# YuyangSunshine/ABR_IOD

Hardware: AMD Instinct MI355X
Metric: training images/sec (R50-C4 Faster R-CNN + ARD) (higher is better)
Workload: dtype f32 (tensors, accumulation and error bound; contractions via a 2-term fp16 split of both operands scaled by their amax, 3 cross products on the fp16 matrix cores: f16x3)

## Files before the change

abr_iod_amd/_lib.py:

```python
import ctypes as C
import os

import torch

_HERE = os.path.dirname(os.path.abspath(__file__))
LIB_PATH = os.environ.get("ABR_IOD_HIP_LIB") or os.path.join(_HERE, "libabr_iod_hip.so")

NCHW, NHWC = 0, 1

_vp, _i, _f, _i64 = C.c_void_p, C.c_int, C.c_float, C.c_int64


class ConvDesc(C.Structure):

    _fields_ = [
        ("B", _i), ("H", _i), ("W", _i), ("Cin", _i),
        ("Cout", _i), ("R", _i), ("S", _i),
        ("stride", _i), ("pad", _i),
        ("Ho", _i), ("Wo", _i),
        ("scale", _vp), ("bias", _vp), ("residual", _vp), ("mask", _vp),
        ("relu", _i),
        ("out_H", _i), ("out_W", _i), ("out_sh", _i), ("out_sw", _i),
        ("math", _i),
        ("wino_v", _vp),
# ... 81 lines not shown
    "abr_deform_psroi_backward": (_i, [_vp, _vp, _vp, _vp, _vp, _vp, _i, _i, _i, _i, _i, _f, _i, _i, _i, _i, _i, _f, _i, _i, _vp, _vp, _vp, _vp]),
    "abr_nms_workspace_bytes": (_i64, [_i, _i]),
    "abr_nms_unsorted_workspace_bytes": (_i64, [_i]),
    "abr_nms": (_i, [_vp, _vp, _i, _f, _i, _vp, _vp, _vp, _i64, _vp]),
    "abr_sort_scores_max_n": (_i64, []),
    "abr_sort_scores_desc": (_i, [_vp, _i, _vp, _vp]),
    "abr_nms_sorted_batched": (_i, [_vp, _vp, _i, _i, _f, _i, _i, _vp, _vp, _vp, _i64, _vp]),
    "abr_roi_align_forward_f64": (_i, [_vp, _vp, _i, _i, _i, _i, _i, C.c_double, _i, _i, _i, _vp, _vp]),
    "abr_roi_align_backward_f64": (_i, [_vp, _vp, _i, _i, _i, _i, _i, C.c_double, _i, _i, _i, _vp, _vp]),
    "abr_sigmoid_focal_forward_f64": (_i, [_vp, _vp, _i, _i, _f, _f, _vp, _vp]),
    "abr_sigmoid_focal_backward_f64": (_i, [_vp, _vp, _vp, _i, _i, _f, _f, _vp, _vp]),
    "abr_sigmoid_focal_forward": (_i, [_vp, _vp, _i, _i, _f, _f, _vp, _vp]),
    "abr_sigmoid_focal_backward": (_i, [_vp, _vp, _vp, _i, _i, _f, _f, _vp, _vp]),
    "abr_ard_forward": (_i, [_vp, _vp, _i, _i, _i, _f, _i, _vp, _vp, _vp]),
    "abr_ard_backward": (_i, [_vp, _vp, _vp, _i, _i, _i, _f, _i, _f, _vp, _vp, _vp]),
    "abr_smooth_l1": (_i, [_vp, _vp, _i64, _f, _f, _vp, _f, _vp, _vp]),
    "abr_smooth_l1_rows": (_i, [_vp, _i, _vp, _vp, _vp, _vp, _i, _f, _f, _vp, _vp, _f, _vp, _vp]),
    "abr_softmax_ce": (_i, [_vp, _i, _vp, _i, _i, _i, _i, _vp, _f, _vp, _i, _vp]),
    "abr_feat_distill": (_i, [_vp, _vp, _i64, _vp, _vp, _f, _vp, _vp]),
    "abr_rpn_distill": (_i, [_vp, _vp, _i, _i, _vp, _vp, _i, _i, _i64, _i, _f, _i, _vp, _f, _vp, _vp, _i, _i, _vp]),
    "abr_roi_distill": (_i, [_vp, _vp, _vp, _vp, _i, _i, _i, _vp, _i, _vp, _f, _vp, _vp, _vp]),
    "abr_bce_logits_gather": (_i, [_vp, _vp, _vp, _vp, _i, _vp, _vp, _f, _vp, _vp]),
    "abr_img_resample_u8": (_i, [_vp, _i, _i, _vp, _i, _i, _vp, _vp, _i, _vp, _vp, _i, _vp, _vp]),
    "abr_img_blend_paste_u8": (_i, [_vp, _i, _i, _vp, _i, _i, _i, _i, _i, _i, _i, _i, C.c_double, _vp]),
    "abr_img_copy_rect_u8": (_i, [_vp, _i, _i, _vp, _i, _i, _i, _i, _i, _i, _i, _i, _vp]),
    "abr_img_fill_u8": (_i, [_vp, _i64, _i, _vp]),
    "abr_img_color_jitter_u8": (_i, [_vp, _i, _i, _i, C.c_double, _vp, _vp]),
    "abr_img_normalize_to_batch": (_i, [_vp, _i, _i, _i, _i, C.POINTER(C.c_float), C.POINTER(C.c_float), _vp, _i, _i, _vp]),
    "abr_conv_forward": (_i, [C.POINTER(ConvDesc), _vp, _vp, _vp, _vp]),
    "abr_conv_tail64_forward": (_i, [C.POINTER(ConvDesc), C.POINTER(ConvDesc), _vp, _vp, _vp, _vp, _vp]),
    "abr_conv_wgrad": (_i, [C.POINTER(ConvDesc), _vp, _vp, _vp, _vp]),
    "abr_conv_wino_v_floats": (_i64, [C.POINTER(ConvDesc)]),
    "abr_conv_route_info": (_i, [C.POINTER(ConvDesc), C.POINTER(C.c_int32)]),
    "abr_conv_packed_bytes": (_i64, [_i64, _i64]),
    "abr_conv_pack_weights": (_i, [_vp, _i64, _i, _vp, _vp]),
    "abr_conv_dgrad_weights": (_i, [_vp, _vp, _i, _i, _i, _i, _vp, _vp]),
    "abr_bias_grad": (_i, [_vp, _i64, _i, _vp, _vp]),
    "abr_nchw_to_nhwc_pad": (_i, [_vp, _i, _i, _i, _i, _i, _vp, _vp]),
    "abr_nchw_to_nhwc": (_i, [_vp, _i, _i, _i, _i, _vp, _vp]),
    "abr_nhwc_to_nchw": (_i, [_vp, _i, _i, _i, _i, _vp, _vp]),
    "abr_maxpool3x3s2": (_i, [_vp, _i, _i, _i, _i, _vp, _vp]),
    "abr_maxpool3x3s2_backward": (_i, [_vp, _vp, _i, _i, _i, _i, _vp, _vp]),
    "abr_deform_im2col": (_i, [_vp, _vp, _i, _i, _i, _i, _i, _i, _i, _vp, _vp]),
    "abr_deform_col2im_coord": (_i, [_vp, _vp, _vp, _i, _i, _i, _i, _i, _i, _i, _vp, _vp, _vp, C.c_uint32, _vp]),
    "abr_deform_im2col_general": (_i, [_vp, _vp, _vp] + [_i] * 16 + [_vp, _vp]),
    "abr_deform_col2im_coord_general": (_i, [_vp, _vp, _vp, _vp] + [_i] * 16 + [_vp, _vp, _vp, _vp]),
    "abr_avgpool_forward": (_i, [_vp, _i, _i, _i, _vp, _vp]),
    "abr_avgpool_backward": (_i, [_vp, _i, _i, _i, _vp, _vp]),
    "abr_avgpool_relu_backward": (_i, [_vp, _vp, _i, _i, _i, _vp, _vp]),
    "abr_avgpool_relu_backward_amax": (_i, [_vp, _vp, _i, _i, _i, _vp, _vp, C.c_uint32, _vp]),
    "abr_channel_mean": (_i, [_vp, _i64, _i, _vp, _vp]),
    "abr_relu_backward": (_i, [_vp, _vp, _i64, _vp, _vp]),
    "abr_add_inplace": (_i, [_vp, _vp, _i64, _vp]),
    "abr_scale_inplace": (_i, [_vp, _i64, _f, _vp, _vp]),
    "abr_grid_anchors": (_i, [_vp, _i, _i, _i, _i, _i, _i, _i, _vp, _vp, _vp]),
    "abr_topk_sigmoid": (_i, [_vp, _i64, _i, _i, _i, _i, _i, _vp, _vp, _vp]),
    "abr_det_softmax_decode": (_i, [_vp, _i, _vp, _i, _i, _i, _vp, _i, _i, _vp, _f, _f, _f, _f, _vp, _vp, _vp]),
    "abr_det_select_workspace_bytes": (_i64, [_i, _i, _i]),
    "abr_det_select": (_i, [_vp, _vp, _vp, _i, _i, _i, _f, _f, _i, _i, _vp, _vp, _vp, _vp, _vp, _vp, _vp, _vp, _i64, _vp]),
    "abr_rpn_decode_clip": (_i, [_vp, _i, _i, _i, _vp, _vp, _i, _i, _i, _vp, _f, _f, _f, _f, _vp, _vp]),
    "abr_rpn_pyramid_max_k": (_i, []),
    "abr_rpn_pyramid_topk": (_i, [_vp, _vp, _vp, _vp, _i, _i, _i, _i, _vp, _vp, _vp]),
    "abr_rpn_pyramid_decode": (_i, [_vp, _vp, _vp, _vp, _vp, _i, _i, _i, _i, _vp, _vp, _vp, _f, _f, _f, _f, _f, _vp, _vp, _vp, _vp]),
    "abr_rpn_pyramid_select": (_i, [_vp, _vp, _vp, _vp, _i, _i, _i, _i, _i, _i, _vp, _vp, _vp, _vp, _vp]),
    "abr_retina_max_candidates": (_i, []),
    "abr_retina_detect": (_i, [_vp, _vp, _vp, _vp, _vp, _vp, _i, _i, _i, _i, _vp, _f, _i, _f, _i, _f, _f, _f, _f, _f, _i, _vp, _vp, _vp, _vp, _vp]),
# ... 114 lines not shown
```

abr_iod_amd/csrc/conv_winograd.hip:

```cpp
#include <map>

#include <algorithm>
#include <map>
#include <functional>
#include <mutex>
#include <utility>
#include <type_traits>
#include <vector>

#include "common.h"

namespace {

template <int V>
struct vf {
    float v[V];
};
template <int V>
__device__ __forceinline__ vf<V> operator+(vf<V> a, vf<V> b) {
    vf<V> r;
#pragma unroll
    for (int i = 0; i < V; i++) r.v[i] = a.v[i] + b.v[i];
    return r;
}
template <int V>
__device__ __forceinline__ vf<V> operator-(vf<V> a, vf<V> b) {
    vf<V> r;
#pragma unroll
    for (int i = 0; i < V; i++) r.v[i] = a.v[i] - b.v[i];
    return r;
}
template <int V>
__device__ __forceinline__ vf<V> operator-(vf<V> a) {
    vf<V> r;
#pragma unroll
// ... 7 lines not shown
    for (int i = 0; i < V; i++) r.v[i] = s * a.v[i];
    return r;
}
template <int V>
__device__ __forceinline__ vf<V> vzero() {
    vf<V> r;
#pragma unroll
    for (int i = 0; i < V; i++) r.v[i] = 0.f;
    return r;
}
template <int V>
__device__ __forceinline__ vf<V> vld(const float* p);
template <>
__device__ __forceinline__ vf<2> vld<2>(const float* p) { const float2 t = *reinterpret_cast<const float2*>(p); return {{t.x, t.y}}; }
template <>
__device__ __forceinline__ vf<4> vld<4>(const float* p) { const float4 t = *reinterpret_cast<const float4*>(p); return {{t.x, t.y, t.z, t.w}}; }
template <int V>
__device__ __forceinline__ vf<V> vld_buf(__amdgpu_buffer_rsrc_t r, unsigned byte_off);
template <>
__device__ __forceinline__ vf<2> vld_buf<2>(__amdgpu_buffer_rsrc_t r, unsigned byte_off) {
    typedef unsigned u32x2 __attribute__((ext_vector_type(2)));
    const u32x2 t = __builtin_amdgcn_raw_buffer_load_b64(r, (int)byte_off, 0, 0);
    return {{__uint_as_float(t.x), __uint_as_float(t.y)}};
}
template <>
__device__ __forceinline__ vf<4> vld_buf<4>(__amdgpu_buffer_rsrc_t r, unsigned byte_off) {
    typedef unsigned u32x4 __attribute__((ext_vector_type(4)));
    const u32x4 t = __builtin_amdgcn_raw_buffer_load_b128(r, (int)byte_off, 0, 0);
    return {{__uint_as_float(t.x), __uint_as_float(t.y), __uint_as_float(t.z), __uint_as_float(t.w)}};
}
__device__ __forceinline__ void vst(float* p, vf<2> a) { *reinterpret_cast<float2*>(p) = make_float2(a.v[0], a.v[1]); }
__device__ __forceinline__ void vst(float* p, vf<4> a) { *reinterpret_cast<float4*>(p) = make_float4(a.v[0], a.v[1], a.v[2], a.v[3]); }

template <typename T>
__device__ __forceinline__ void bt6(const T d0, const T d1, const T d2, const T d3, const T d4, const T d5, T& o0, T& o1, T& o2, T& o3, T& o4,
                                    T& o5) {
    o0 = 4.f * d0 - 5.f * d2 + d4;
    o1 = d3 + d4 - 4.f * (d1 + d2);
    o2 = 4.f * d1 - 4.f * d2 - d3 + d4;
    o3 = 2.f * (d3 - d1) - d2 + d4;
    o4 = 2.f * d1 - d2 - 2.f * d3 + d4;
    o5 = 4.f * d1 - 5.f * d3 + d5;
}

template <int V>
__device__ __forceinline__ unsigned vabs_max(unsigned m, vf<V> a) {
#pragma unroll
    for (int i = 0; i < V; i++) m = max(m, __float_as_uint(a.v[i]) & 0x7FFFFFFFu);
    return m;
}

template <int V>
__global__ __launch_bounds__(256) void wino_input_kernel(const float* __restrict__ x, int B, int H, int W, int C, int th_n, int tw_n,
                                                         float* __restrict__ Vo, unsigned long long* amax, unsigned epoch) {
    unsigned am = 0;
    typedef vf<V> f2;
    const int64_t T = (int64_t)B * th_n * tw_n;
    const int C2 = C / V;
    const int64_t total = T * C2;
    const int64_t ps = T * C;
    const __amdgpu_buffer_rsrc_t rx = __builtin_amdgcn_make_buffer_rsrc(const_cast<float*>(x), 0, (unsigned)((int64_t)B * H * W * C * 4), 0x00020000);
    for (int64_t idx = (int64_t)blockIdx.x * blockDim.x + threadIdx.x; idx < total; idx += (int64_t)gridDim.x * blockDim.x) {
        const int c = V * (int)(idx % C2);
        const int64_t t = idx / C2;
        const int tw = (int)(t % tw_n), th = (int)((t / tw_n) % th_n), b = (int)(t / ((int64_t)tw_n * th_n));
        const int y0 = 4 * th - 1, x0 = 4 * tw - 1;
        f2 tcol[6][6];
        const int base = (b * H * W) * C + c;
#pragma unroll
        for (int j = 0; j < 6; j++) {
            const int xx = x0 + j;
            const bool xin = (unsigned)xx < (unsigned)W;
            f2 d[6];
#pragma unroll
            for (int i = 0; i < 6; i++) {
// ... 161 lines not shown
            const float4 a = *reinterpret_cast<const float4*>(src + (r * 3 + q) * 64), b = *reinterpret_cast<const float4*>(src + (r * 3 + q) * 64 + 4);
            gA[r][q] = {{a.x, a.y, a.z, a.w}};
            gB[r][q] = {{b.x, b.y, b.z, b.w}};
        }
    uint4* planes = reinterpret_cast<uint4*>(jb.dst);
    const float* scales = reinterpret_cast<const float*>(reinterpret_cast<const char*>(jb.dst) + abr::h3_planes_bytes_dev(36 * N, C));
    const int ks = kc * 4 + wave, KS = C / 16;
    auto emit = [&](int xi, const fv& uA, const fv& uB, float sc) {
        const float inv = 1.f / sc;
        unsigned h0[4], h1[4];
        abr::h3_split2(uA.v[0], uA.v[1], inv, h0[0], h1[0]);
        abr::h3_split2(uA.v[2], uA.v[3], inv, h0[1], h1[1]);
        abr::h3_split2(uB.v[0], uB.v[1], inv, h0[2], h1[2]);
        abr::h3_split2(uB.v[2], uB.v[3], inv, h0[3], h1[3]);
        const size_t nb = ((size_t)xi * N + n0) / 32;
        const size_t ch = (nb * KS + ks) * 2;
        planes[ch * 64 + lane] = make_uint4(h0[0], h0[1], h0[2], h0[3]);
        planes[(ch + 1) * 64 + lane] = make_uint4(h1[0], h1[1], h1[2], h1[3]);
    };
    auto row_i = [&](auto I) {
        constexpr int i = decltype(I)::value;
        float sc[6];
#pragma unroll
        for (int jj = 0; jj < 6; jj++) sc[jj] = scales[(size_t)(6 * i + jj) * N + n0 + row];
        fv uA[6], uB[6];
        wino_u_row<i>(gA, uA);
        wino_u_row<i>(gB, uB);
#pragma unroll
        for (int jj = 0; jj < 6; jj++) emit(6 * i + jj, uA[jj], uB[jj], sc[jj]);
    };
    for_rows6(row_i);
}

template <typename T>
__device__ __forceinline__ void at4(const T m0, const T m1, const T m2, const T m3, const T m4, const T m5, T& o0, T& o1, T& o2, T& o3) {
    const T s12 = m1 + m2, d12 = m1 - m2, s34 = m3 + m4, d34 = m3 - m4;
    o0 = m0 + s12 + s34;
    o1 = d12 + 2.f * d34;
    o2 = s12 + 4.f * s34;
    o3 = d12 + 8.f * d34 + m5;
}

template <int V>
__global__ __launch_bounds__(256) void wino_output_kernel(const float* __restrict__ Mm, int B, int H, int W, int N, int th_n, int tw_n,
                                                          const float* __restrict__ scale, const float* __restrict__ bias, int relu,
                                                          const float* __restrict__ mask, float* __restrict__ out, unsigned long long* amax, unsigned epoch) {
    typedef vf<V> f2;
    unsigned am = 0;
    const int64_t T = (int64_t)B * th_n * tw_n;
    const int N2 = N / V;
    const int64_t total = T * N2;
    const int64_t ps = T * N;
    for (int64_t idx = (int64_t)blockIdx.x * blockDim.x + threadIdx.x; idx < total; idx += (int64_t)gridDim.x * blockDim.x) {
        const int n = V * (int)(idx % N2);
        const int64_t t = idx / N2;
        const int tw = (int)(t % tw_n), th = (int)((t / tw_n) % th_n), b = (int)(t / ((int64_t)tw_n * th_n));
        const float* m = Mm + t * N + n;
        f2 tcol[4][6];
#pragma unroll
        for (int j = 0; j < 6; j++)
            at4(vld<V>(m + (0 + j) * ps), vld<V>(m + (6 + j) * ps), vld<V>(m + (12 + j) * ps), vld<V>(m + (18 + j) * ps), vld<V>(m + (24 + j) * ps),
                vld<V>(m + (30 + j) * ps), tcol[0][j], tcol[1][j], tcol[2][j], tcol[3][j]);
        f2 sc, bi;
#pragma unroll
        for (int e = 0; e < V; e++) { sc.v[e] = scale ? scale[n + e] : 1.f; bi.v[e] = bias ? bias[n + e] : 0.f; }
        f2 mk[4][4];
        if (mask) {
#pragma unroll
            for (int i = 0; i < 4; i++)
#pragma unroll
                for (int j = 0; j < 4; j++) {
                    const int oy = 4 * th + i, ox = 4 * tw + j;
                    const bool in = oy < H && ox < W;
                    mk[i][j] = vld<V>(mask + (((int64_t)b * H + (in ? oy : 4 * th)) * W + (in ? ox : 4 * tw)) * N + n);
                }
        }
#pragma unroll
        for (int i = 0; i < 4; i++) {
            f2 y[4];
            at4(tcol[i][0], tcol[i][1], tcol[i][2], tcol[i][3], tcol[i][4], tcol[i][5], y[0], y[1], y[2], y[3]);
            const int oy = 4 * th + i;
            if (oy >= H) continue;
#pragma unroll
            for (int j = 0; j < 4; j++) {
                const int ox = 4 * tw + j;
                if (ox >= W) continue;
                const int64_t o = (((int64_t)b * H + oy) * W + ox) * N + n;
                f2 v;
#pragma unroll
                for (int e = 0; e < V; e++) {
                    v.v[e] = y[j].v[e] * sc.v[e] + bi.v[e];
                    if (relu) v.v[e] = abr::relu_f(v.v[e]);
                }
                if (mask) {
#pragma unroll
                    for (int e = 0; e < V; e++) v.v[e] = mk[i][j].v[e] > 0.f ? v.v[e] : 0.f;
                }
                vst(out + o, v);
                if (amax) am = vabs_max(am, v);
            }
        }
    }
    if (amax) abr::h3_amax_emit(amax, epoch, am);
}

template <typename T>
__device__ __forceinline__ void a6(const T y0, const T y1, const T y2, const T y3, T& o0, T& o1, T& o2, T& o3, T& o4, T& o5) {
    o0 = y0;
    o1 = y0 + y1 + y2 + y3;
    o2 = y0 - y1 + y2 - y3;
    o3 = y0 + 2.f * y1 + 4.f * y2 + 8.f * y3;
    o4 = y0 - 2.f * y1 + 4.f * y2 - 8.f * y3;
    o5 = y3;
}

template <int V>
__global__ __launch_bounds__(256) void wino_outgrad_kernel(const float* __restrict__ gy, int B, int H, int W, int N, int th_n, int tw_n,
                                                           float* __restrict__ Mg, unsigned long long* amax, unsigned epoch) {
    typedef vf<V> f2;
    unsigned am = 0;
    const int64_t T = (int64_t)B * th_n * tw_n;
    const int N2 = N / V;
    const int64_t total = T * N2;
    const int64_t ps = T * N;
    for (int64_t idx = (int64_t)blockIdx.x * blockDim.x + threadIdx.x; idx < total; idx += (int64_t)gridDim.x * blockDim.x) {
        const int n = V * (int)(idx % N2);
        const int64_t t = idx / N2;
        const int tw = (int)(t % tw_n), th = (int)((t / tw_n) % th_n), b = (int)(t / ((int64_t)tw_n * th_n));
        f2 tcol[6][4];
#pragma unroll
        for (int j = 0; j < 4; j++) {
            const int ox = 4 * tw + j;
            f2 y[4];
#pragma unroll
            for (int i = 0; i < 4; i++) {
                const int oy = 4 * th + i;
                y[i] = (oy < H && ox < W) ? vld<V>(gy + (((int64_t)b * H + oy) * W + ox) * N + n) : vzero<V>();
            }
            a6(y[0], y[1], y[2], y[3], tcol[0][j], tcol[1][j], tcol[2][j], tcol[3][j], tcol[4][j], tcol[5][j]);
        }
#pragma unroll
        for (int i = 0; i < 6; i++) {
            f2 v0, v1, v2, v3, v4, v5;
            a6(tcol[i][0], tcol[i][1], tcol[i][2], tcol[i][3], v0, v1, v2, v3, v4, v5);
            float* o = Mg + ((int64_t)(6 * i) * T + t) * N + n;
            vst(o, v0); vst(o + ps, v1); vst(o + 2 * ps, v2); vst(o + 3 * ps, v3); vst(o + 4 * ps, v4); vst(o + 5 * ps, v5);
            if (amax) am = vabs_max(vabs_max(vabs_max(vabs_max(vabs_max(vabs_max(am, v0), v1), v2), v3), v4), v5);
        }
    }
    if (amax) abr::h3_amax_emit(amax, epoch, am);
}

template <typename T>
__device__ __forceinline__ void gt3(const T u0, const T u1, const T u2, const T u3, const T u4, const T u5, T& o0, T& o1, T& o2) {
    o0 = 0.25f * u0 - (1.f / 6.f) * (u1 + u2) + (1.f / 24.f) * (u3 + u4);
    o1 = (1.f / 6.f) * (u2 - u1) + (1.f / 12.f) * (u3 - u4);
    o2 = (1.f / 6.f) * (u3 + u4 - u1 - u2) + u5;
}

template <int V>
__global__ __launch_bounds__(256) void wino_wgrad_inverse_kernel(const float* __restrict__ dU, int N, int C, const float* __restrict__ scale,
                                                                 float* __restrict__ dw) {
    typedef vf<V> fv;
    const int Cv = C / V;
    const int64_t total = (int64_t)N * Cv;
    const int64_t ps = (int64_t)N * C;
    for (int64_t idx = (int64_t)blockIdx.x * blockDim.x + threadIdx.x; idx < total; idx += (int64_t)gridDim.x * blockDim.x) {
        const int c = V * (int)(idx % Cv);
        const int64_t n = idx / Cv;
        const float* u = dU + n * C + c;
        fv tcol[3][6];
#pragma unroll
        for (int j = 0; j < 6; j++)
            gt3(vld<V>(u + (0 + j) * ps), vld<V>(u + (6 + j) * ps), vld<V>(u + (12 + j) * ps), vld<V>(u + (18 + j) * ps), vld<V>(u + (24 + j) * ps),
                vld<V>(u + (30 + j) * ps), tcol[0][j], tcol[1][j], tcol[2][j]);
        const float sc = scale ? scale[n] : 1.f;
        fv old[3][3];
#pragma unroll
        for (int r = 0; r < 3; r++)
#pragma unroll
            for (int q = 0; q < 3; q++) old[r][q] = vld<V>(dw + ((n * 3 + r) * 3 + q) * C + c);
#pragma unroll
        for (int r = 0; r < 3; r++) {
            fv g0, g1, g2;
            gt3(tcol[r][0], tcol[r][1], tcol[r][2], tcol[r][3], tcol[r][4], tcol[r][5], g0, g1, g2);
            float* o = dw + ((n * 3 + r) * 3) * C + c;
            vst(o, old[r][0] + sc * g0); vst(o + C, old[r][1] + sc * g1); vst(o + 2 * C, old[r][2] + sc * g2);
        }
    }
}

inline unsigned grid_for(int64_t n) { return (unsigned)std::min<int64_t>((n + 255) / 256, 32768); }
inline unsigned grid_for(int64_t n, bool) { return grid_for(n); }

}

namespace abr {

static inline bool wide(int64_t tiles, int C) {
    return C % 4 == 0 && tiles * (C / 4) >= (int64_t)256 * 4 * 256;
}

int wino_input_transform(const float* x, int B, int H, int W, int C, float* V, hipStream_t st, const AmaxRef* amax) {
    const int th_n = (H + 3) / 4, tw_n = (W + 3) / 4;
    unsigned long long* aw = amax ? amax->word : nullptr;
    const unsigned ae = amax ? amax->epoch : 0u;
    wino_input_kernel<2><<<grid_for((int64_t)B * th_n * tw_n * (C / 2), aw != nullptr), 256, 0, st>>>(x, B, H, W, C, th_n, tw_n, V, aw, ae);
    return hipGetLastError() == hipSuccess ? 0 : 1;
}

void prep_wino_h3_direct(const PrepJobs& jobs, int pack_blocks, int scale_blocks, unsigned* flags, hipStream_t st) {
    if (!jobs.n) return;
    static std::once_flag attr_once;
    std::call_once(attr_once, [] {
        (void)hipFuncSetAttribute(reinterpret_cast<const void*>(wino_h3_pack_multi_kernel<PrepTable>), hipFuncAttributeMaxDynamicSharedMemorySize, (int)kWhLds);
        (void)hipFuncSetAttribute(reinterpret_cast<const void*>(wino_h3_pack_multi_kernel<PrepJob>), hipFuncAttributeMaxDynamicSharedMemorySize, (int)kWhLds);
    });
    prep_each(jobs, [&](auto src) {
        wino_h3_scales_multi_kernel<<<(unsigned)scale_blocks, 256, 0, st>>>(src, flags);
        wino_h3_pack_multi_kernel<<<(unsigned)pack_blocks, 256, kWhLds, st>>>(src);
    });
}

void prep_wino_u(const PrepJobs& jobs, int blocks, hipStream_t st) {
    prep_each(jobs, [&](auto src) { wino_weight_multi_kernel<<<(unsigned)blocks, 256, 0, st>>>(src); });
}

int wino_output_transform(const float* Mm, int B, int H, int W, int N, const float* scale, const float* bias, int relu, const float* mask,
                          float* out, hipStream_t st, const AmaxRef* amax) {
    const int th_n = (H + 3) / 4, tw_n = (W + 3) / 4;
    unsigned long long* aw = amax ? amax->word : nullptr;
    const unsigned ae = amax ? amax->epoch : 0u;
    if (wide((int64_t)B * th_n * tw_n, N))
        wino_output_kernel<4><<<grid_for((int64_t)B * th_n * tw_n * (N / 4), aw != nullptr), 256, 0, st>>>(Mm, B, H, W, N, th_n, tw_n, scale, bias, relu, mask, out, aw, ae);
    else
        wino_output_kernel<2><<<grid_for((int64_t)B * th_n * tw_n * (N / 2), aw != nullptr), 256, 0, st>>>(Mm, B, H, W, N, th_n, tw_n, scale, bias, relu, mask, out, aw, ae);
    return hipGetLastError() == hipSuccess ? 0 : 1;
}

int wino_outgrad_transform(const float* gy, int B, int H, int W, int N, float* Mg, hipStream_t st, const AmaxRef* amax) {
    const int th_n = (H + 3) / 4, tw_n = (W + 3) / 4;
    unsigned long long* aw = amax ? amax->word : nullptr;
    const unsigned ae = amax ? amax->epoch : 0u;
    if (wide((int64_t)B * th_n * tw_n, N)) wino_outgrad_kernel<4><<<grid_for((int64_t)B * th_n * tw_n * (N / 4), aw != nullptr), 256, 0, st>>>(gy, B, H, W, N, th_n, tw_n, Mg, aw, ae);
    else wino_outgrad_kernel<2><<<grid_for((int64_t)B * th_n * tw_n * (N / 2), aw != nullptr), 256, 0, st>>>(gy, B, H, W, N, th_n, tw_n, Mg, aw, ae);
    return hipGetLastError() == hipSuccess ? 0 : 1;
}

int wino_wgrad_inverse(const float* dU, int N, int C, const float* scale, float* dw, hipStream_t st) {
    if (C % 4 == 0) wino_wgrad_inverse_kernel<4><<<grid_for((int64_t)N * (C / 4)), 256, 0, st>>>(dU, N, C, scale, dw);
    else wino_wgrad_inverse_kernel<2><<<grid_for((int64_t)N * (C / 2)), 256, 0, st>>>(dU, N, C, scale, dw);
    return hipGetLastError() == hipSuccess ? 0 : 1;
}

namespace {
struct DEntry {
    void* buf = nullptr; size_t bytes = 0; int64_t version = 0; hipStream_t stream = nullptr; hipEvent_t filled = nullptr;
    std::vector<hipStream_t> readers;
    uint64_t last_use = 0;
    int64_t pending = 0;
};
std::map<std::pair<const void*, int>, DEntry> g_dcache;
std::mutex g_dcache_mu;
uint64_t g_dcache_clock = 0;
size_t g_dcache_bytes = 0;

void dcache_drop(DEntry& e) {
    if (e.stream) (void)hipStreamSynchronize(e.stream);
    for (hipStream_t r : e.readers) (void)hipStreamSynchronize(r);
    if (e.buf) { (void)hipFree(e.buf); g_dcache_bytes -= e.bytes; }
    if (e.filled) (void)hipEventDestroy(e.filled);
    e = DEntry();
}
size_t dcache_limit() {
    static const size_t mb = getenv("ABR_WINO_CACHE_MB") ? (size_t)atoll(getenv("ABR_WINO_CACHE_MB")) : 4096;
    return mb << 20;
}
// ... 90 lines not shown
    for (int i = 0; i < n; i++) {
        DEntry* e = reinterpret_cast<DEntry*>(tokens[i]);
        if (!e) continue;
        e->pending = 0;
        e->version = 0;
    }
}

void derived_cache_clear() {
    std::lock_guard<std::mutex> lock(g_dcache_mu);
    for (auto it = g_dcache.begin(); it != g_dcache.end();) {
        if (it->second.pending) { ++it; continue; }
        dcache_drop(it->second);
        it = g_dcache.erase(it);
    }
}
void derived_cache_drop_range(const void* base, size_t bytes) {
    std::lock_guard<std::mutex> lock(g_dcache_mu);
    const char* lo = reinterpret_cast<const char*>(base);
    const char* hi = lo + bytes;
    for (auto it = g_dcache.begin(); it != g_dcache.end();) {
        const char* k = reinterpret_cast<const char*>(it->first.first);
        if (k < lo || k >= hi || it->second.pending) { ++it; continue; }
        dcache_drop(it->second);
        it = g_dcache.erase(it);
    }
}
size_t derived_cache_bytes() {
    std::lock_guard<std::mutex> lock(g_dcache_mu);
    return g_dcache_bytes;
}

}
```

include/abr_iod_hip.h:

```cpp
#ifndef ABR_IOD_HIP_H
#define ABR_IOD_HIP_H

#include <stdint.h>

#ifdef __cplusplus
extern "C" {
#endif

#define ABR_OK 0
#define ABR_E_INVALID (-1)
#define ABR_E_LAUNCH (-2)
#define ABR_E_WORKSPACE (-3)

#define ABR_NCHW 0
#define ABR_NHWC 1

const char* abr_last_error(void);
int abr_version(void);
int abr_device_info(int32_t* out_host);

int abr_prof_begin(void);
int abr_prof_mark_overlap(int on);
int abr_stream_wait_stream(void* waiter, void* signaller);
int abr_prof_set_mask(uint32_t id_mask, int every_nth);
// ... 172 lines not shown
int abr_conv_forward(const abr_conv_desc* d_host, const float* x, const float* w, float* out, void* stream);
int abr_conv_tail64_forward(const abr_conv_desc* d2_host, const abr_conv_desc* d3_host, const float* x, const float* w2, const float* w3, float* out,
                            void* stream);
int abr_conv_prepare_weights(const float* w, int Cout, int R, int S, int Cin, int stride, int pad, int math, int64_t w_version, void* stream);
typedef struct abr_prep_item {
    const float* w;
    const float* scale;
    float* wt;
    int32_t Cout, R, S, Cin, stride, pad, math;
    int64_t w_version;
} abr_prep_item;
int abr_conv_prepare_batch(const abr_prep_item* items_host, int n, void* stream);

#define ABR_OP_FORWARD 0
#define ABR_OP_WGRAD 1
#define ABR_OP_STREAM_WAIT 2
typedef struct abr_conv_op {
    int32_t kind;
    int32_t reserved;
    abr_conv_desc desc;
    const float* a;
    const float* b;
    float* out;
    void* stream;
    void* other;
} abr_conv_op;
int abr_conv_run(const abr_conv_op* ops, int n);
int abr_conv_cache_clear(void);
int abr_conv_cache_drop_range(const void* base, int64_t bytes);
int64_t abr_conv_cache_bytes(void);
int64_t abr_scratch_bytes(void);
int64_t abr_conv_wino_v_floats(const abr_conv_desc* d_host);
int abr_conv_route_info(const abr_conv_desc* d_host, int32_t out[4]);
int64_t abr_conv_packed_bytes(int64_t rows, int64_t K);
int abr_conv_pack_weights(const float* w, int64_t rows, int K, void* planes, void* stream);

int abr_conv_wgrad(const abr_conv_desc* d_host, const float* x, const float* gy, float* dw, void* stream);

int abr_conv_dgrad_weights(const float* w, const float* scale, int Cout, int R, int S, int Cin, float* wt,
                           void* stream);
int abr_bias_grad(const float* gy, int64_t M, int C, float* db, void* stream);

int abr_nchw_to_nhwc_pad(const float* x, int B, int C, int H, int W, int Cpad, float* out, void* stream);
int abr_nhwc_to_nchw(const float* x, int B, int C, int H, int W, float* out, void* stream);
int abr_nchw_to_nhwc(const float* x, int B, int C, int H, int W, float* out, void* stream);
int abr_maxpool3x3s2(const float* x, int B, int H, int W, int C, float* out, void* stream);
int abr_maxpool3x3s2_backward(const float* y, const float* g_pool, int B, int H, int W, int C, float* g_y, void* stream);
int abr_deform_im2col(const float* x, const float* om, int B, int H, int W, int C, int Com, int dg, int modulated, float* cols, void* stream);
int abr_deform_col2im_coord(const float* dcol, const float* x, const float* om, int B, int H, int W, int C, int Com, int dg, int modulated,
                            float* dx, float* d_om, uint64_t* d_om_amax, uint32_t d_om_amax_epoch, void* stream);
int abr_deform_im2col_general(const float* x, const float* offset, const float* mask, int B, int H, int W, int C, int Ho, int Wo, int kh, int kw,
                              int stride_h, int stride_w, int pad_h, int pad_w, int dil_h, int dil_w, int groups, int dg, float* cols,
                              void* stream);
int abr_deform_col2im_coord_general(const float* dcol, const float* x, const float* offset, const float* mask, int B, int H, int W, int C, int Ho,
                                    int Wo, int kh, int kw, int stride_h, int stride_w, int pad_h, int pad_w, int dil_h, int dil_w, int groups,
                                    int dg, float* dx, float* d_offset, float* d_mask, void* stream);
int abr_avgpool_forward(const float* x, int N, int HW, int C, float* out, void* stream);
int abr_avgpool_backward(const float* g, int N, int HW, int C, float* gx, void* stream);
int abr_avgpool_relu_backward(const float* g, const float* y, int N, int HW, int C, float* gx, void* stream);
int abr_avgpool_relu_backward_amax(const float* g, const float* y, int N, int HW, int C, float* gx, uint64_t* amax, uint32_t amax_epoch, void* stream);
int abr_channel_mean(const float* x, int64_t rows, int C, float* out, void* stream);
int abr_relu_backward(const float* g, const float* y, int64_t n, float* out, void* stream);
int abr_add_inplace(float* a, const float* b, int64_t n, void* stream);
int abr_loss_sum(const float* const* terms_host, const float* weights_host, const int32_t* groups_host, int n, float* total, float* out,
                 void* stream);
int abr_loss_sum_backward(const float* weights_host, int n, const float* g, float* grads, void* stream);
// ... 170 lines not shown
```

Before: 230.9.

## Add LDS-staged Winograd input/output/outgrad transforms sharing row transforms across tiles

Adds shared-memory variants of the Winograd F(4,3) input, output and output-gradient transform kernels. Each block first applies the row transform to a strip of columns, stages the result in LDS, then applies the column transform. Overlapping tile columns are therefore loaded and transformed once rather than per tile, which cuts redundant global reads and arithmetic. A heuristic picks a strip width of 4 or 8 tiles by grid size. The change also rewrites the transform helpers with explicit FMA ordering and fp contraction disabled so the old and new paths round identically, and adds C entry points for standalone transform calls and a copy yardstick for benchmarking. The risks are LDS-limited occupancy and extra synchronization on small grids.

New measurement: 228.3. 0.989x the previous value.

```diff
diff --git a/abr_iod_amd/_lib.py b/abr_iod_amd/_lib.py
--- a/abr_iod_amd/_lib.py
+++ b/abr_iod_amd/_lib.py
@@ -137,6 +137,11 @@
     "abr_conv_wgrad": (_i, [C.POINTER(ConvDesc), _vp, _vp, _vp, _vp]),
     "abr_conv_wino_v_floats": (_i64, [C.POINTER(ConvDesc)]),
     "abr_conv_route_info": (_i, [C.POINTER(ConvDesc), C.POINTER(C.c_int32)]),
+    "abr_wino_lds_mode": (_i, [_i]),
+    "abr_wino_input_transform": (_i, [_vp, _i, _i, _i, _i, _vp, _vp, C.c_uint32, _vp]),
+    "abr_wino_output_transform": (_i, [_vp, _i, _i, _i, _i, _vp, _vp, _i, _vp, _vp, _vp, C.c_uint32, _vp]),
+    "abr_wino_outgrad_transform": (_i, [_vp, _i, _i, _i, _i, _vp, _vp, C.c_uint32, _vp]),
+    "abr_wino_copy_yardstick": (_i, [_vp, _i64, _vp, _i64, _vp]),
     "abr_conv_packed_bytes": (_i64, [_i64, _i64]),
     "abr_conv_pack_weights": (_i, [_vp, _i64, _i, _vp, _vp]),
     "abr_conv_dgrad_weights": (_i, [_vp, _vp, _i, _i, _i, _i, _vp, _vp]),
diff --git a/abr_iod_amd/csrc/conv_winograd.hip b/abr_iod_amd/csrc/conv_winograd.hip
--- a/abr_iod_amd/csrc/conv_winograd.hip
+++ b/abr_iod_amd/csrc/conv_winograd.hip
@@ -1,6 +1,7 @@
 #include <map>
 
 #include <algorithm>
+#include <atomic>
 #include <map>
 #include <functional>
 #include <mutex>
@@ -74,15 +75,21 @@
 __device__ __forceinline__ void vst(float* p, vf<2> a) { *reinterpret_cast<float2*>(p) = make_float2(a.v[0], a.v[1]); }
 __device__ __forceinline__ void vst(float* p, vf<4> a) { *reinterpret_cast<float4*>(p) = make_float4(a.v[0], a.v[1], a.v[2], a.v[3]); }
 
-template <typename T>
-__device__ __forceinline__ void bt6(const T d0, const T d1, const T d2, const T d3, const T d4, const T d5, T& o0, T& o1, T& o2, T& o3, T& o4,
-                                    T& o5) {
-    o0 = 4.f * d0 - 5.f * d2 + d4;
-    o1 = d3 + d4 - 4.f * (d1 + d2);
-    o2 = 4.f * d1 - 4.f * d2 - d3 + d4;
-    o3 = 2.f * (d3 - d1) - d2 + d4;
-    o4 = 2.f * d1 - d2 - 2.f * d3 + d4;
-    o5 = 4.f * d1 - 5.f * d3 + d5;
+template <int V>
+__device__ __forceinline__ void bt6(const vf<V> d0, const vf<V> d1, const vf<V> d2, const vf<V> d3, const vf<V> d4, const vf<V> d5, vf<V>& o0,
+                                    vf<V>& o1, vf<V>& o2, vf<V>& o3, vf<V>& o4, vf<V>& o5) {
+#pragma clang fp contract(off)
+#pragma unroll
+    for (int e = 0; e < V; e++) {
+        const float a0 = d0.v[e], a1 = d1.v[e], a2 = d2.v[e], a3 = d3.v[e], a4 = d4.v[e], a5 = d5.v[e];
+        o0.v[e] = __builtin_fmaf(a0, 4.f, -(a2 * 5.f)) + a4;
+        o1.v[e] = (a3 + a4) - (a1 + a2) * 4.f;
+        o2.v[e] = (__builtin_fmaf(a1, 4.f, -(a2 * 4.f)) - a3) + a4;
+        const float t = a3 - a1;
+        o3.v[e] = ((t + t) - a2) + a4;
+        o4.v[e] = __builtin_fmaf(a3, -2.f, __builtin_fmaf(a1, 2.f, -a2)) + a4;
+        o5.v[e] = __builtin_fmaf(a3, -5.f, a1 * 4.f) + a5;
+    }
 }
 
 template <int V>
@@ -310,13 +317,31 @@
     for_rows6(row_i);
 }
 
-template <typename T>
-__device__ __forceinline__ void at4(const T m0, const T m1, const T m2, const T m3, const T m4, const T m5, T& o0, T& o1, T& o2, T& o3) {
-    const T s12 = m1 + m2, d12 = m1 - m2, s34 = m3 + m4, d34 = m3 - m4;
-    o0 = m0 + s12 + s34;
-    o1 = d12 + 2.f * d34;
-    o2 = s12 + 4.f * s34;
-    o3 = d12 + 8.f * d34 + m5;
+template <int V>
+__device__ __forceinline__ void at4(const vf<V> m0, const vf<V> m1, const vf<V> m2, const vf<V> m3, const vf<V> m4, const vf<V> m5, vf<V>& o0,
+                                    vf<V>& o1, vf<V>& o2, vf<V>& o3) {
+#pragma clang fp contract(off)
+#pragma unroll
+    for (int e = 0; e < V; e++) {
+        const float s12 = m1.v[e] + m2.v[e], d12 = m1.v[e] - m2.v[e], s34 = m3.v[e] + m4.v[e], d34 = m3.v[e] - m4.v[e];
+        o0.v[e] = (m0.v[e] + s12) + s34;
+        o1.v[e] = __builtin_fmaf(d34, 2.f, d12);
+        o2.v[e] = __builtin_fmaf(s34, 4.f, s12);
+        o3.v[e] = __builtin_fmaf(d34, 8.f, d12) + m5.v[e];
+    }
+}
+
+template <int V>
+__device__ __forceinline__ vf<V> wino_epilogue(const vf<V> y, const vf<V> sc, const vf<V> bi, int relu, bool masked, const vf<V> mk) {
+#pragma clang fp contract(off)
+    vf<V> v;
+#pragma unroll
+    for (int e = 0; e < V; e++) {
+        v.v[e] = __builtin_fmaf(y.v[e], sc.v[e], bi.v[e]);
+        if (relu) v.v[e] = abr::relu_f(v.v[e]);
+        if (masked) v.v[e] = mk.v[e] > 0.f ? v.v[e] : 0.f;
+    }
+    return v;
 }
 
 template <int V>
@@ -364,16 +389,7 @@
                 const int ox = 4 * tw + j;
                 if (ox >= W) continue;
                 const int64_t o = (((int64_t)b * H + oy) * W + ox) * N + n;
-                f2 v;
-#pragma unroll
-                for (int e = 0; e < V; e++) {
-                    v.v[e] = y[j].v[e] * sc.v[e] + bi.v[e];
-                    if (relu) v.v[e] = abr::relu_f(v.v[e]);
-                }
-                if (mask) {
-#pragma unroll
-                    for (int e = 0; e < V; e++) v.v[e] = mk[i][j].v[e] > 0.f ? v.v[e] : 0.f;
-                }
+                const f2 v = wino_epilogue(y[j], sc, bi, relu, mask != nullptr, mask ? mk[i][j] : sc);
                 vst(out + o, v);
                 if (amax) am = vabs_max(am, v);
             }
@@ -382,14 +398,20 @@
     if (amax) abr::h3_amax_emit(amax, epoch, am);
 }
 
-template <typename T>
-__device__ __forceinline__ void a6(const T y0, const T y1, const T y2, const T y3, T& o0, T& o1, T& o2, T& o3, T& o4, T& o5) {
-    o0 = y0;
-    o1 = y0 + y1 + y2 + y3;
-    o2 = y0 - y1 + y2 - y3;
-    o3 = y0 + 2.f * y1 + 4.f * y2 + 8.f * y3;
-    o4 = y0 - 2.f * y1 + 4.f * y2 - 8.f * y3;
-    o5 = y3;
+template <int V>
+__device__ __forceinline__ void a6(const vf<V> y0, const vf<V> y1, const vf<V> y2, const vf<V> y3, vf<V>& o0, vf<V>& o1, vf<V>& o2, vf<V>& o3,
+                                   vf<V>& o4, vf<V>& o5) {
+#pragma clang fp contract(off)
+#pragma unroll
+    for (int e = 0; e < V; e++) {
+        const float a0 = y0.v[e], a1 = y1.v[e], a2 = y2.v[e], a3 = y3.v[e];
+        o0.v[e] = a0;
+        o1.v[e] = ((a0 + a1) + a2) + a3;
+        o2.v[e] = ((a0 - a1) + a2) - a3;
+        o3.v[e] = __builtin_fmaf(a3, 8.f, __builtin_fmaf(a2, 4.f, __builtin_fmaf(a1, 2.f, a0)));
+        o4.v[e] = __builtin_fmaf(-a3, 8.f, __builtin_fmaf(a2, 4.f, __builtin_fmaf(-a1, 2.f, a0)));
+        o5.v[e] = a3;
+    }
 }
 
 template <int V>
@@ -429,6 +451,199 @@
     if (amax) abr::h3_amax_emit(amax, epoch, am);
 }
 
+constexpr int kLdsCh = 64, kLdsC4 = kLdsCh / 4;
+
+struct LdsBlock { int cc, twc, th, b; };
+template <int TWB>
+__device__ __forceinline__ LdsBlock lds_block(int C, int th_n, int tw_n) {
+    const int cc_n = (C + kLdsCh - 1) / kLdsCh, twc_n = (tw_n + TWB - 1) / TWB;
+    int bid = (int)blockIdx.x;
+    LdsBlock k;
+    k.cc = bid % cc_n; bid /= cc_n;
+    k.twc = bid % twc_n; bid /= twc_n;
+    k.th = bid % th_n;
+    k.b = bid / th_n;
+    return k;
+}
+
+template <int TWB>
+__global__ __launch_bounds__(256) void wino_input_lds_kernel(const float* __restrict__ x, int B, int H, int W, int C, int th_n, int tw_n,
+                                                             float* __restrict__ Vo, unsigned long long* amax, unsigned epoch) {
+    typedef vf<4> fv;
+    constexpr int NCOL = 4 * TWB + 2, N1 = NCOL * kLdsC4, IT1 = (N1 + 255) / 256, N2 = 6 * TWB * kLdsC4, IT2 = (N2 + 255) / 256;
+    __shared__ float S[6 * NCOL * kLdsCh];
+    const LdsBlock k = lds_block<TWB>(C, th_n, tw_n);
+    const int tid = (int)threadIdx.x, c4 = tid & (kLdsC4 - 1), c = k.cc * kLdsCh + 4 * c4;
+    const bool cin = c < C;
+    const int64_t T = (int64_t)B * th_n * tw_n, ps = T * C;
+    const __amdgpu_buffer_rsrc_t rx = __builtin_amdgcn_make_buffer_rsrc(const_cast<float*>(x), 0, (unsigned)((int64_t)B * H * W * C * 4), 0x00020000);
+    const int y0 = 4 * k.th - 1, xb = 4 * TWB * k.twc - 1;
+    const int base = (k.b * H * W) * C + c;
+    fv d[IT1][6];
+#pragma unroll
+    for (int it = 0; it < IT1; it++) {
+        const int item = tid + 256 * it, xx = xb + (item >> 4);
+        const bool ok = item < N1 && cin && (unsigned)xx < (unsigned)W;
+#pragma unroll
+        for (int i = 0; i < 6; i++) {
+            const int y = y0 + i;
+            d[it][i] = vld_buf<4>(rx, ok && (unsigned)y < (unsigned)H ? (unsigned)(base + (y * W + xx) * C) * 4u : 0x80000000u);
+        }
+    }
+#pragma unroll
+    for (int it = 0; it < IT1; it++) {
+        const int item = tid + 256 * it;
+        if (item < N1) {
+            fv t[6];
+            bt6(d[it][0], d[it][1], d[it][2], d[it][3], d[it][4], d[it][5], t[0], t[1], t[2], t[3], t[4], t[5]);
+#pragma unroll
+            for (int i = 0; i < 6; i++) vst(S + (i * NCOL) * kLdsCh + item * 4, t[i]);
+        }
+    }
+    __syncthreads();
+    unsigned am = 0;
+#pragma unroll
+    for (int it = 0; it < IT2; it++) {
+        const int item = tid + 256 * it, twl = (item >> 4) % TWB, i = item / (kLdsC4 * TWB), tw = k.twc * TWB + twl;
+        if (item < N2 && cin && tw < tw_n) {
+            const float* s = S + ((i * NCOL + 4 * twl) * kLdsC4 + c4) * 4;
+            fv v0, v1, v2, v3, v4, v5;
+            bt6(vld<4>(s), vld<4>(s + kLdsCh), vld<4>(s + 2 * kLdsCh), vld<4>(s + 3 * kLdsCh), vld<4>(s + 4 * kLdsCh), vld<4>(s + 5 * kLdsCh), v0, v1, v2,
+                v3, v4, v5);
+            const int64_t t = ((int64_t)k.b * th_n + k.th) * tw_n + tw;
+            float* o = Vo + ((int64_t)(6 * i) * T + t) * C + c;
+            vst(o, v0); vst(o + ps, v1); vst(o + 2 * ps, v2); vst(o + 3 * ps, v3); vst(o + 4 * ps, v4); vst(o + 5 * ps, v5);
+            if (amax) am = vabs_max(vabs_max(vabs_max(vabs_max(vabs_max(vabs_max(am, v0), v1), v2), v3), v4), v5);
+        }
+    }
+    if (amax) abr::h3_amax_emit(amax, epoch, am);
+}
+
+template <int TWB>
+__global__ __launch_bounds__(256) void wino_output_lds_kernel(const float* __restrict__ Mm, int B, int H, int W, int N, int th_n, int tw_n,
+                                                              const float* __restrict__ scale, const float* __restrict__ bias, int relu,
+                                                              const float* __restrict__ mask, float* __restrict__ out, unsigned long long* amax,
+                                                              unsigned epoch) {
+    typedef vf<4> fv;
+    constexpr int N1 = 6 * TWB * kLdsC4, IT1 = (N1 + 255) / 256, N2 = 4 * TWB * kLdsC4, IT2 = (N2 + 255) / 256;
+    __shared__ float S[4 * TWB * 6 * kLdsCh];
+    const LdsBlock k = lds_block<TWB>(N, th_n, tw_n);
+    const int tid = (int)threadIdx.x, c4 = tid & (kLdsC4 - 1), n = k.cc * kLdsCh + 4 * c4;
+    const bool nin = n < N;
+    const int64_t T = (int64_t)B * th_n * tw_n, ps = T * N;
+    const int64_t t0 = ((int64_t)k.b * th_n + k.th) * tw_n + (int64_t)k.twc * TWB;
+    fv m[IT1][6];
+#pragma unroll
+    for (int it = 0; it < IT1; it++) {
+        const int item = tid + 256 * it, twl = (item >> 4) % TWB, j = item / (kLdsC4 * TWB);
+        const bool ok = item < N1 && nin && k.twc * TWB + twl < tw_n;
+        const float* p = Mm + (t0 + twl) * N + n + j * ps;
+#pragma unroll
+        for (int i = 0; i < 6; i++) m[it][i] = ok ? vld<4>(p + (6 * i) * ps) : vzero<4>();
+    }
+    fv mk[IT2][4], sc, bi;
+#pragma unroll
+    for (int e = 0; e < 4; e++) { sc.v[e] = scale && nin ? scale[n + e] : 1.f; bi.v[e] = bias && nin ? bias[n + e] : 0.f; }
+#pragma unroll
+    for (int it = 0; it < IT2; it++) {
+        const int item = tid + 256 * it, twl = (item >> 4) % TWB, i = item / (kLdsC4 * TWB), tw = k.twc * TWB + twl, oy = 4 * k.th + i;
+        const bool ok = mask && item < N2 && nin && tw < tw_n && oy < H;
+#pragma unroll
+        for (int j = 0; j < 4; j++) mk[it][j] = ok && 4 * tw + j < W ? vld<4>(mask + (((int64_t)k.b * H + oy) * W + 4 * tw + j) * N + n) : vzero<4>();
+    }
+#pragma unroll
+    for (int it = 0; it < IT1; it++) {
+        const int item = tid + 256 * it, twl = (item >> 4) % TWB, j = item / (kLdsC4 * TWB);
+        if (item < N1) {
+            fv t[4];
+            at4(m[it][0], m[it][1], m[it][2], m[it][3], m[it][4], m[it][5], t[0], t[1], t[2], t[3]);
+#pragma unroll
+            for (int i = 0; i < 4; i++) vst(S + (((i * TWB + twl) * 6 + j) * kLdsC4 + c4) * 4, t[i]);
+        }
+    }
+    __syncthreads();
+    unsigned am = 0;
+#pragma unroll
+    for (int it = 0; it < IT2; it++) {
+        const int item = tid + 256 * it, twl = (item >> 4) % TWB, i = item / (kLdsC4 * TWB), tw = k.twc * TWB + twl, oy = 4 * k.th + i;
+        if (item < N2 && nin && tw < tw_n && oy < H) {
+            const float* s = S + (((i * TWB + twl) * 6) * kLdsC4 + c4) * 4;
+            fv y[4];
+            at4(vld<4>(s), vld<4>(s + kLdsCh), vld<4>(s + 2 * kLdsCh), vld<4>(s + 3 * kLdsCh), vld<4>(s + 4 * kLdsCh), vld<4>(s + 5 * kLdsCh), y[0], y[1],
+                y[2], y[3]);
+#pragma unroll
+            for (int j = 0; j < 4; j++) {
+                const int ox = 4 * tw + j;
+                if (ox >= W) continue;
+                const fv v = wino_epilogue(y[j], sc, bi, relu, mask != nullptr, mk[it][j]);
+                vst(out + (((int64_t)k.b * H + oy) * W + ox) * N + n, v);
+                if (amax) am = vabs_max(am, v);
+            }
+        }
+    }
+    if (amax) abr::h3_amax_emit(amax, epoch, am);
+}
+
+template <int TWB>
+__global__ __launch_bounds__(256) void wino_outgrad_lds_kernel(const float* __restrict__ gy, int B, int H, int W, int N, int th_n, int tw_n,
+                                                               float* __restrict__ Mg, unsigned long long* amax, unsigned epoch) {
+    typedef vf<4> fv;
+    constexpr int N1 = 4 * TWB * kLdsC4, IT1 = (N1 + 255) / 256, N2 = 6 * TWB * kLdsC4, IT2 = (N2 + 255) / 256;
+    __shared__ float S[6 * TWB * 4 * kLdsCh];
+    const LdsBlock k = lds_block<TWB>(N, th_n, tw_n);
+    const int tid = (int)threadIdx.x, c4 = tid & (kLdsC4 - 1), n = k.cc * kLdsCh + 4 * c4;
+    const bool nin = n < N;
+    const int64_t T = (int64_t)B * th_n * tw_n, ps = T * N;
+    fv g[IT1][4];
+#pragma unroll
+    for (int it = 0; it < IT1; it++) {
+        const int item = tid + 256 * it, ox = 4 * TWB * k.twc + (item >> 4);
+        const bool ok = item < N1 && nin && ox < W;
+#pragma unroll
+        for (int i = 0; i < 4; i++) {
+            const int oy = 4 * k.th + i;
+            g[it][i] = ok && oy < H ? vld<4>(gy + (((int64_t)k.b * H + oy) * W + ox) * N + n) : vzero<4>();
+        }
+    }
+#pragma unroll
+    for (int it = 0; it < IT1; it++) {
+        const int item = tid + 256 * it, col = item >> 4;
+        if (item < N1) {
+            fv t[6];
+            a6(g[it][0], g[it][1], g[it][2], g[it][3], t[0], t[1], t[2], t[3], t[4], t[5]);
+#pragma unroll
+            for (int i = 0; i < 6; i++) vst(S + ((i * TWB * 4 + col) * kLdsC4 + c4) * 4, t[i]);
+        }
+    }
+    __syncthreads();
+    unsigned am = 0;
+#pragma unroll
+    for (int it = 0; it < IT2; it++) {
+        const int item = tid + 256 * it, twl = (item >> 4) % TWB, i = item / (kLdsC4 * TWB), tw = k.twc * TWB + twl;
+        if (item < N2 && nin && tw < tw_n) {
+            const float* s = S + ((i * TWB * 4 + 4 * twl) * kLdsC4 + c4) * 4;
+            fv v0, v1, v2, v3, v4, v5;
+            a6(vld<4>(s), vld<4>(s + kLdsCh), vld<4>(s + 2 * kLdsCh), vld<4>(s + 3 * kLdsCh), v0, v1, v2, v3, v4, v5);
+            const int64_t t = ((int64_t)k.b * th_n + k.th) * tw_n + tw;
+            float* o = Mg + ((int64_t)(6 * i) * T + t) * N + n;
+            vst(o, v0); vst(o + ps, v1); vst(o + 2 * ps, v2); vst(o + 3 * ps, v3); vst(o + 4 * ps, v4); vst(o + 5 * ps, v5);
+            if (amax) am = vabs_max(vabs_max(vabs_max(vabs_max(vabs_max(vabs_max(am, v0), v1), v2), v3), v4), v5);
+        }
+    }
+    if (amax) abr::h3_amax_emit(amax, epoch, am);
+}
+
+__global__ __launch_bounds__(256) void wino_copy_yardstick_kernel(const float4* __restrict__ src, int64_t n_src, float4* __restrict__ dst, int64_t n_dst) {
+    const int64_t stride = (int64_t)gridDim.x * blockDim.x, i0 = (int64_t)blockIdx.x * blockDim.x + threadIdx.x;
+    const int64_t both = n_src < n_dst ? n_src : n_dst;
+    float4 v = make_float4(0.f, 0.f, 0.f, 0.f);
+    for (int64_t i = i0; i < both; i += stride) { v = src[i]; dst[i] = v; }
+    for (int64_t i = both + i0; i < n_dst; i += stride) dst[i] = v;
+    float acc = 0.f;
+    for (int64_t i = both + i0; i < n_src; i += stride) { const float4 t = src[i]; acc += t.x + t.y + t.z + t.w; }
+    if (acc == 1.2345e-30f && n_dst) dst[0].x = acc;
+}
+
 template <typename T>
 __device__ __forceinline__ void gt3(const T u0, const T u1, const T u2, const T u3, const T u4, const T u5, T& o0, T& o1, T& o2) {
     o0 = 0.25f * u0 - (1.f / 6.f) * (u1 + u2) + (1.f / 24.f) * (u3 + u4);
@@ -479,11 +694,27 @@
     return C % 4 == 0 && tiles * (C / 4) >= (int64_t)256 * 4 * 256;
 }
 
+static std::atomic<int> g_wino_lds_mode{1};
+static inline int lds_form(bool won, int B, int th_n, int tw_n, int C, int twb_small_grid = 4) {
+    const int mode = g_wino_lds_mode.load(std::memory_order_relaxed);
+    if (mode == 0 || (mode == 1 && !won) || C % 4 != 0 || C < 4) return 0;
+    const int64_t grid4 = (int64_t)B * th_n * ((tw_n + 3) / 4) * ((C + kLdsCh - 1) / kLdsCh);
+    if (grid4 > 0x7FFFFFFF) return 0;
+    if (mode == 1) return grid4 < 1024 ? twb_small_grid : 4;
+    return mode == 8 ? 8 : 4;
+}
+static inline unsigned lds_grid(int twb, int B, int th_n, int tw_n, int C) {
+    return (unsigned)((int64_t)B * th_n * ((tw_n + twb - 1) / twb) * ((C + kLdsCh - 1) / kLdsCh));
+}
+
 int wino_input_transform(const float* x, int B, int H, int W, int C, float* V, hipStream_t st, const AmaxRef* amax) {
     const int th_n = (H + 3) / 4, tw_n = (W + 3) / 4;
     unsigned long long* aw = amax ? amax->word : nullptr;
     const unsigned ae = amax ? amax->epoch : 0u;
-    wino_input_kernel<2><<<grid_for((int64_t)B * th_n * tw_n * (C / 2), aw != nullptr), 256, 0, st>>>(x, B, H, W, C, th_n, tw_n, V, aw, ae);
+    const int twb = lds_form(tw_n >= 4, B, th_n, tw_n, C);
+    if (twb == 8) wino_input_lds_kernel<8><<<lds_grid(8, B, th_n, tw_n, C), 256, 0, st>>>(x, B, H, W, C, th_n, tw_n, V, aw, ae);
+    else if (twb == 4) wino_input_lds_kernel<4><<<lds_grid(4, B, th_n, tw_n, C), 256, 0, st>>>(x, B, H, W, C, th_n, tw_n, V, aw, ae);
+    else wino_input_kernel<2><<<grid_for((int64_t)B * th_n * tw_n * (C / 2), aw != nullptr), 256, 0, st>>>(x, B, H, W, C, th_n, tw_n, V, aw, ae);
     return hipGetLastError() == hipSuccess ? 0 : 1;
 }
 
@@ -509,7 +740,12 @@
     const int th_n = (H + 3) / 4, tw_n = (W + 3) / 4;
     unsigned long long* aw = amax ? amax->word : nullptr;
     const unsigned ae = amax ? amax->epoch : 0u;
-    if (wide((int64_t)B * th_n * tw_n, N))
+    const int twb = lds_form(tw_n >= 4, B, th_n, tw_n, N, 8);
+    if (twb == 8)
+        wino_output_lds_kernel<8><<<lds_grid(8, B, th_n, tw_n, N), 256, 0, st>>>(Mm, B, H, W, N, th_n, tw_n, scale, bias, relu, mask, out, aw, ae);
+    else if (twb == 4)
+        wino_output_lds_kernel<4><<<lds_grid(4, B, th_n, tw_n, N), 256, 0, st>>>(Mm, B, H, W, N, th_n, tw_n, scale, bias, relu, mask, out, aw, ae);
+    else if (wide((int64_t)B * th_n * tw_n, N))
         wino_output_kernel<4><<<grid_for((int64_t)B * th_n * tw_n * (N / 4), aw != nullptr), 256, 0, st>>>(Mm, B, H, W, N, th_n, tw_n, scale, bias, relu, mask, out, aw, ae);
     else
         wino_output_kernel<2><<<grid_for((int64_t)B * th_n * tw_n * (N / 2), aw != nullptr), 256, 0, st>>>(Mm, B, H, W, N, th_n, tw_n, scale, bias, relu, mask, out, aw, ae);
@@ -520,7 +756,10 @@
     const int th_n = (H + 3) / 4, tw_n = (W + 3) / 4;
     unsigned long long* aw = amax ? amax->word : nullptr;
     const unsigned ae = amax ? amax->epoch : 0u;
-    if (wide((int64_t)B * th_n * tw_n, N)) wino_outgrad_kernel<4><<<grid_for((int64_t)B * th_n * tw_n * (N / 4), aw != nullptr), 256, 0, st>>>(gy, B, H, W, N, th_n, tw_n, Mg, aw, ae);
+    const int twb = lds_form(tw_n >= 4 && !wide((int64_t)B * th_n * tw_n, N), B, th_n, tw_n, N);
+    if (twb == 8) wino_outgrad_lds_kernel<8><<<lds_grid(8, B, th_n, tw_n, N), 256, 0, st>>>(gy, B, H, W, N, th_n, tw_n, Mg, aw, ae);
+    else if (twb == 4) wino_outgrad_lds_kernel<4><<<lds_grid(4, B, th_n, tw_n, N), 256, 0, st>>>(gy, B, H, W, N, th_n, tw_n, Mg, aw, ae);
+    else if (wide((int64_t)B * th_n * tw_n, N)) wino_outgrad_kernel<4><<<grid_for((int64_t)B * th_n * tw_n * (N / 4), aw != nullptr), 256, 0, st>>>(gy, B, H, W, N, th_n, tw_n, Mg, aw, ae);
     else wino_outgrad_kernel<2><<<grid_for((int64_t)B * th_n * tw_n * (N / 2), aw != nullptr), 256, 0, st>>>(gy, B, H, W, N, th_n, tw_n, Mg, aw, ae);
     return hipGetLastError() == hipSuccess ? 0 : 1;
 }
@@ -677,3 +916,41 @@
 }
 
 }
+
+extern "C" int abr_wino_lds_mode(int mode) {
+    const int old = abr::g_wino_lds_mode.load();
+    if (mode == 0 || mode == 1 || mode == 4 || mode == 8) abr::g_wino_lds_mode.store(mode);
+    return old;
+}
+static bool wino_shape_ok(int B, int H, int W, int C) {
+    return B > 0 && H > 0 && W > 0 && C > 0 && C % 2 == 0 && (int64_t)B * H * W * C * 4 < ((int64_t)1 << 31);
+}
+extern "C" int abr_wino_input_transform(const float* x, int B, int H, int W, int C, float* V, uint64_t* amax, uint32_t epoch, void* stream) {
+    ABR_REQUIRE(x && V && wino_shape_ok(B, H, W, C), "wino_input_transform: needs pointers, an even C and an input below 2 GB");
+    const abr::AmaxRef ref{reinterpret_cast<unsigned long long*>(amax), epoch};
+    ABR_REQUIRE(!abr::wino_input_transform(x, B, H, W, C, V, abr::as_stream(stream), amax ? &ref : nullptr), "wino_input_transform: launch failed");
+    return ABR_OK;
+}
+extern "C" int abr_wino_output_transform(const float* M, int B, int H, int W, int N, const float* scale, const float* bias, int relu,
+                                         const float* mask, float* out, uint64_t* amax, uint32_t epoch, void* stream) {
+    ABR_REQUIRE(M && out && wino_shape_ok(B, H, W, N), "wino_output_transform: needs pointers, an even N and an output below 2 GB");
+    const abr::AmaxRef ref{reinterpret_cast<unsigned long long*>(amax), epoch};
+    ABR_REQUIRE(!abr::wino_output_transform(M, B, H, W, N, scale, bias, relu, mask, out, abr::as_stream(stream), amax ? &ref : nullptr),
+                "wino_output_transform: launch failed");
+    return ABR_OK;
+}
+extern "C" int abr_wino_outgrad_transform(const float* gy, int B, int H, int W, int N, float* Mg, uint64_t* amax, uint32_t epoch, void* stream) {
+    ABR_REQUIRE(gy && Mg && wino_shape_ok(B, H, W, N), "wino_outgrad_transform: needs pointers, an even N and a gradient below 2 GB");
+    const abr::AmaxRef ref{reinterpret_cast<unsigned long long*>(amax), epoch};
+    ABR_REQUIRE(!abr::wino_outgrad_transform(gy, B, H, W, N, Mg, abr::as_stream(stream), amax ? &ref : nullptr), "wino_outgrad_transform: launch failed");
+    return ABR_OK;
+}
+extern "C" int abr_wino_copy_yardstick(const void* src, int64_t src_bytes, void* dst, int64_t dst_bytes, void* stream) {
+    ABR_REQUIRE(src && dst && src_bytes >= 0 && dst_bytes >= 0 && src_bytes % 16 == 0 && dst_bytes % 16 == 0, "wino_copy_yardstick: bad args");
+    const int64_t n = std::max(src_bytes, dst_bytes) / 16;
+    if (!n) return ABR_OK;
+    wino_copy_yardstick_kernel<<<(unsigned)std::min<int64_t>((n + 255) / 256, 256 * 8), 256, 0, abr::as_stream(stream)>>>(
+        static_cast<const float4*>(src), src_bytes / 16, static_cast<float4*>(dst), dst_bytes / 16);
+    ABR_CHECK_LAUNCH("wino_copy_yardstick");
+    return ABR_OK;
+}
diff --git a/include/abr_iod_hip.h b/include/abr_iod_hip.h
--- a/include/abr_iod_hip.h
+++ b/include/abr_iod_hip.h
@@ -228,6 +228,12 @@
 int64_t abr_scratch_bytes(void);
 int64_t abr_conv_wino_v_floats(const abr_conv_desc* d_host);
 int abr_conv_route_info(const abr_conv_desc* d_host, int32_t out[4]);
+int abr_wino_lds_mode(int mode);
+int abr_wino_input_transform(const float* x, int B, int H, int W, int C, float* V, uint64_t* amax, uint32_t epoch, void* stream);
+int abr_wino_output_transform(const float* M, int B, int H, int W, int N, const float* scale, const float* bias, int relu, const float* mask,
+                              float* out, uint64_t* amax, uint32_t epoch, void* stream);
+int abr_wino_outgrad_transform(const float* gy, int B, int H, int W, int N, float* Mg, uint64_t* amax, uint32_t epoch, void* stream);
+int abr_wino_copy_yardstick(const void* src, int64_t src_bytes, void* dst, int64_t dst_bytes, void* stream);
 int64_t abr_conv_packed_bytes(int64_t rows, int64_t K);
 int abr_conv_pack_weights(const float* w, int64_t rows, int K, void* planes, void* stream);
 
```
